# tum-vision/dvo_slam

Measured on AMD Instinct MI355X. Metric: frame-pair alignments/s (640x480, 4-level pyramid) + finest-level HBM GB/s vs roofline, higher is better.
Workload: dtype f32 (Gram operands exact f16 hi + lo pairs on every level, f32 accumulate); 1 GPU; 1024 pairs (BASELINE config 4): independent 640x480 RGB-D frame pairs, seeds 0..1023, pair i on rank i mod 1, 4-level pyramid, FirstLevel=3, LastLevel=0, MaxIterationsPerLevel=100, Precision=5e-7, Mu=0; step = every rank re-ingests the raw planes of its shard from HBM (pyramids, sampling planes, point selection) and aligns it as one batch; the build of step k+1 (build stream) overlaps the match of; pairs=1024, pairs_per_gpu=1024, width=640, height=480, lanes=1 lane

## Files before the change

dvo_slam_amd/csrc/align_coarse.hip:

```cpp
#include "fast_sweep.h"
#include "mfma_sweep.h"
#include "solver_logic.h"

namespace dvo_hip {

namespace {

__device__ __forceinline__ int coarse_uniform(int v) { return __builtin_amdgcn_readfirstlane(v); }
__device__ __forceinline__ float coarse_uniform(float v) { return __builtin_bit_cast(float, __builtin_amdgcn_readfirstlane(__builtin_bit_cast(int, v))); }

template <typename T>
__device__ __forceinline__ void coarse_copy(T* dst, const T* src) {
  static_assert(sizeof(T) % 4 == 0, "POD must be a multiple of 4 bytes");
  const unsigned* s = reinterpret_cast<const unsigned*>(src);
  unsigned* d = reinterpret_cast<unsigned*>(dst);
  for (int i = threadIdx.x; i < int(sizeof(T) / 4); i += kBlock) d[i] = s[i];
}

constexpr int kCoarseReduceInFlight = 8;
constexpr int kCoarseLlSlots = 4, kCoarseLlLoads = 4;

}

template <int WG_PER_CU>
// ... 37 lines not shown
    const int tiles = g.tiles_x * g.tiles_y;
    const bool window_level = !g.linear && g.compact;
    float* my_partials = a.partials + size_t(pair) * a.max_tiles * kAccStride;
    float2* my_residuals = a.scratch + size_t(pair) * a.max_entries;
    int* my_flag = a.f16_range_flag ? a.f16_range_flag + pair : nullptr;

    for (;;) {
      float KT[12], Pp[4];
#pragma unroll
      for (int i = 0; i < 12; ++i) KT[i] = coarse_uniform(st.KT[i]);
#pragma unroll
      for (int i = 0; i < 4; ++i) Pp[i] = coarse_uniform(st.P_prev[i]);
      const bool first = coarse_uniform(st.first) != 0;
      if (window_level) {
        const FastWeights wt(Pp, first);
        if (g.w % kTileW != 0) {
#pragma unroll 1
          for (int tile = 0; tile < tiles; ++tile)
            fast_sweep_tile<2, true, true, 0, false>(g, KT, wt, pp, 0, tile, my_partials, my_residuals, lds, no_table, a.fallback_count, my_flag);
        } else {
#pragma unroll 1
          for (int tile = 0; tile < tiles; ++tile)
            fast_sweep_tile<2, false, true, 0, false>(g, KT, wt, pp, 0, tile, my_partials, my_residuals, lds, no_table, a.fallback_count, my_flag);
        }
      } else if (g.linear) {
#pragma unroll 1
        for (int tile = 0; tile < tiles; ++tile) {
          mfma_sweep_tile<kCoarseRowsPerWave, true, 2>(g, KT, Pp, first, pp, 0, tile, my_partials, my_residuals, &slab[0][0], counts, my_flag);
          __syncthreads();
        }
      } else {
#pragma unroll 1
        for (int tile = 0; tile < tiles; ++tile) {
          mfma_sweep_tile<kCoarseRowsPerWave, false, 2>(g, KT, Pp, first, pp, 0, tile, my_partials, my_residuals, &slab[0][0], counts, my_flag);
          __syncthreads();
        }
      }
      __syncthreads();
// ... 78 lines not shown
```

dvo_slam_amd/csrc/align_fast.hip:

```cpp
#include "fast_sweep.h"
#include "solver_step.h"

namespace dvo_hip {

template <int STORE, bool PARTIAL, bool COMPACT, int COMPAT, bool HI_J, int TAIL>
__global__ __launch_bounds__(256, COMPAT == 2 ? 4 : 5) void k_sweep_fast(
    const LevelGeom g, const PairPtrs* __restrict__ pairs, const PairState* __restrict__ states, int n_pairs,
    float* __restrict__ partials, float2* __restrict__ scratch, int blocks_per_xcd, unsigned long long* __restrict__ fallback_count, int* __restrict__ f16_range_flag,
    const SolverStepArgs tail) {
  const int tiles = g.tiles_x * g.tiles_y;
  const int total = tiles * n_pairs;
  const int xcd = blockIdx.x & 7, slot = blockIdx.x >> 3;
  const int item = xcd * blocks_per_xcd + slot;
  if (item >= total) return;
  const int entry = item / tiles, tile = item - entry * tiles;
  const int pair = pair_of_launch_index(g, entry);
  if (pair < 0) return;
  const PairState& st = states[pair];
  __shared__ __attribute__((aligned(16))) float slab[4][kSlabFloatsF16];
  __shared__ __attribute__((aligned(16))) float2 win[kFastCells];
  __shared__ __attribute__((aligned(16))) int bbox[4][2];
  __shared__ int counts[4];
  static_assert(TAIL == 0 || sizeof(SweepTailLds) + 16 <= sizeof(win), "the step's LDS lies over the window");
  if (!st.active || st.level != g.level) {
// ... 5 lines not shown
  const FastRcpSource rcp_table = {__builtin_amdgcn_make_buffer_rsrc(const_cast<float*>(COMPAT ? g.rcp_table : nullptr), 0, COMPAT ? (4 << (23 - g.rcp_shift)) : 0, 0x00020000),
                                   rcp_lds, g.rcp_shift};
  if constexpr (COMPAT == 2) {
    const int entries = 1 << (23 - g.rcp_shift);
    const __amdgpu_buffer_rsrc_t packed = __builtin_amdgcn_make_buffer_rsrc(const_cast<float*>(g.rcp_table) + entries, 0, entries * 2, 0x00020000);
    f32x4 chunk[2];
#pragma unroll
    for (int j = 0; j < 2; ++j) chunk[j] = __builtin_bit_cast(f32x4, __builtin_amdgcn_raw_buffer_load_b128(packed, (int(threadIdx.x) + j * 256) * 16, 0, 0));
#pragma unroll
    for (int j = 0; j < 2; ++j)
      if ((int(threadIdx.x) + j * 256) * 8 < entries) reinterpret_cast<f32x4*>(rcp_lds)[threadIdx.x + j * 256] = chunk[j];
    __syncthreads();
  }
  const FastLds lds = {slab, win, bbox, counts};
  const FastWeights wt(st);
  fast_sweep_tile<STORE, PARTIAL, COMPACT, COMPAT, HI_J, TAIL != 0>(g, st.KT, wt, pp, pair, tile, partials, scratch, lds, rcp_table, fallback_count, f16_range_flag);
  if constexpr (TAIL == 1) sweep_tail(g, tail, pair, reinterpret_cast<char*>(win));
  if constexpr (TAIL == 2) sweep_tail_wide(g, tail, pair, reinterpret_cast<char*>(win));
}

bool sweep_fast_has_tail(int variant, const LevelGeom& g) { return variant == 8 && !g.rcp_table && !g.gram_hi_j && fast_sweep_supports(g); }

bool fast_sweep_takes_width(int w) { return w >= kFastCols && w % 2 == 0; }

bool fast_sweep_supports(const LevelGeom& g) {
  const long long plane_bytes = 8ll * g.w * g.h, packed_bytes = 8ll * kCompactTileEntries * g.tiles_x * g.tiles_y;
  return !g.linear && fast_sweep_takes_width(g.w) && g.w < 32768 && g.h < 32768 && plane_bytes < (1ll << 31) && packed_bytes < (1ll << 31);
}

void launch_sweep_fast(hipStream_t s, int variant, const LevelGeom& g, const PairPtrs* pairs, const PairState* states, int n_pairs,
                       float* partials, float2* scratch, unsigned long long* fallback_count, int* f16_range_flag, const SolverStepArgs* tail) {
  const int total = g.tiles_x * g.tiles_y * n_pairs;
  const int per_xcd = (total + 7) / 8;
  const dim3 grid(per_xcd * 8), block(256);
  const bool partial = g.w % kTileW != 0, compact = g.compact != 0;
  const SolverStepArgs no_tail = {};
  if (tail) {
    auto with = [&](auto partial_tag, auto compact_tag) {
      constexpr bool kP = decltype(partial_tag)::value, kC = decltype(compact_tag)::value;
      if (tail->pair_sums) k_sweep_fast<2, kP, kC, 0, false, 2><<<grid, block, 0, s>>>(g, pairs, states, n_pairs, partials, scratch, per_xcd, fallback_count, f16_range_flag, *tail);
      else k_sweep_fast<2, kP, kC, 0, false, 1><<<grid, block, 0, s>>>(g, pairs, states, n_pairs, partials, scratch, per_xcd, fallback_count, f16_range_flag, *tail);
    };
    if (compact) { if (partial) with(std::true_type{}, std::true_type{}); else with(std::false_type{}, std::true_type{}); }
    else { if (partial) with(std::true_type{}, std::false_type{}); else with(std::false_type{}, std::false_type{}); }
    return;
  }
  auto go = [&](auto store_tag, auto partial_tag, auto compact_tag, auto compat_tag) {
    constexpr int kStore = decltype(store_tag)::value;
    if (g.gram_hi_j && kStore == 2)
      k_sweep_fast<2, decltype(partial_tag)::value, decltype(compact_tag)::value, decltype(compat_tag)::value, true, 0>
          <<<grid, block, 0, s>>>(g, pairs, states, n_pairs, partials, scratch, per_xcd, fallback_count, f16_range_flag, no_tail);
    else
      k_sweep_fast<kStore, decltype(partial_tag)::value, decltype(compact_tag)::value, decltype(compat_tag)::value, false, 0>
          <<<grid, block, 0, s>>>(g, pairs, states, n_pairs, partials, scratch, per_xcd, fallback_count, f16_range_flag, no_tail);
  };
  using S1 = std::integral_constant<int, 1>;
  using S2 = std::integral_constant<int, 2>;
  using T = std::true_type;
  using F = std::false_type;
  using C0 = std::integral_constant<int, 0>;
  using C1 = std::integral_constant<int, 1>;
  using C2 = std::integral_constant<int, 2>;
  if (g.rcp_table && g.rcp_packed) {
    if (compact) { if (partial) go(S2{}, T{}, T{}, C2{}); else go(S2{}, F{}, T{}, C2{}); }
    else { if (partial) go(S2{}, T{}, F{}, C2{}); else go(S2{}, F{}, F{}, C2{}); }
  } else if (g.rcp_table) {
    if (compact) { if (partial) go(S2{}, T{}, T{}, C1{}); else go(S2{}, F{}, T{}, C1{}); }
    else { if (partial) go(S2{}, T{}, F{}, C1{}); else go(S2{}, F{}, F{}, C1{}); }
  } else if (variant == 8) {
    if (compact) { if (partial) go(S2{}, T{}, T{}, C0{}); else go(S2{}, F{}, T{}, C0{}); }
    else { if (partial) go(S2{}, T{}, F{}, C0{}); else go(S2{}, F{}, F{}, C0{}); }
  } else {
    if (compact) { if (partial) go(S1{}, T{}, T{}, C0{}); else go(S1{}, F{}, T{}, C0{}); }
    else { if (partial) go(S1{}, T{}, F{}, C0{}); else go(S1{}, F{}, F{}, C0{}); }
  }
}

}
```

dvo_slam_amd/csrc/capi_frames.inc:

```
int stamp_build(dvo_hip_context* ctx, int n, dvo_hip_frame* const* frames) {
  const unsigned long long seq = ++ctx->build_seq;
  DVO_HIP_TRY(ctx, hipEventRecord(ctx->build_events[seq % dvo_hip_context::kBuildRing], ctx->build_stream));
  for (int i = 0; i < n; ++i) frames[i]->built_seq = seq;
  return DVO_HIP_OK;
}

int wait_for_ticket(dvo_hip_context* ctx, unsigned long long need, bool upload) {
  unsigned long long& waited = upload ? ctx->upload_waited_seq : ctx->main_waited_seq;
  hipStream_t stream = upload ? ctx->upload_stream : ctx->stream;
  if (need <= waited) return DVO_HIP_OK;
  const unsigned long long oldest_live = ctx->build_seq >= dvo_hip_context::kBuildRing ? ctx->build_seq - dvo_hip_context::kBuildRing + 1 : 1;
  const unsigned long long use = need < oldest_live ? oldest_live : need;
  DVO_HIP_TRY(ctx, hipStreamWaitEvent(stream, ctx->build_events[use % dvo_hip_context::kBuildRing], 0));
  waited = use;
  return DVO_HIP_OK;
}

int wait_for_build(dvo_hip_context* ctx, int n, dvo_hip_frame* const* frames) {
  unsigned long long need = 0;
  for (int i = 0; i < n; ++i)
    if (frames[i] && frames[i]->built_seq > need) need = frames[i]->built_seq;
  return wait_for_ticket(ctx, need, false);
}

// ... 95 lines not shown
    off += align_up(size_t(c->h[l]) * 4, 256);
    e = hipMemcpy(c->tx[l], host.data(), size_t(c->w[l]) * 4, hipMemcpyHostToDevice);
    if (e == hipSuccess) e = hipMemcpy(c->ty[l], host.data() + c->w[l], size_t(c->h[l]) * 4, hipMemcpyHostToDevice);
    if (e != hipSuccess) {
      c->tables.release();
      delete c;
      ctx->err = std::string("hipMemcpy(camera tables): ") + hipGetErrorString(e);
      return DVO_HIP_ERR_HIP;
    }
  }
  ctx->cameras.push_back(c);
  *out = c;
  return DVO_HIP_OK;
}

void level_tiles(int w, int h, int rows_per_wave, bool linear, int* tiles_x, int* tiles_y) {
  const int th = kWavesPerBlock * rows_per_wave;
  if (linear) {
    const int segments = (w * h + kTileW - 1) / kTileW;
    *tiles_x = 1;
    *tiles_y = (segments + th - 1) / th;
  } else {
    *tiles_x = (w + kTileW - 1) / kTileW;
    *tiles_y = (h + th - 1) / th;
  }
}

bool level_uses_fast_window(const dvo_hip_context* ctx, int w, int h) {
  return ctx->opt_variant >= 8 && fast_sweep_takes_width(w) && w < 32768 && h < 32768;
}

bool level_uses_small(const dvo_hip_context* ctx, int w, int h);

bool level_is_linear(const dvo_hip_context* ctx, int w) { return ctx->opt_variant >= 5 && w % kTileW != 0 && !level_uses_fast_window(ctx, w, 4); }

bool level_uses_window(const dvo_hip_context* ctx, int w, int h) {
  return (ctx->opt_variant >= 6 && w % kTileW == 0 && w < 32768 && h < 32768) || level_uses_fast_window(ctx, w, h);
}
// ... 1 lines not shown
bool level_uses_small(const dvo_hip_context* ctx, int w, int h) {
  return ctx->opt_small_sweep && ctx->opt_variant >= 8 && !ctx->opt_ref_compat && !ctx->opt_ref_order && !level_uses_window(ctx, w, h) && level_is_linear(ctx, w) && small_sweep_takes(w, h);
}

LevelGeom make_geom(const dvo_hip_context* ctx, const CameraGeom* cam, int level, int rows_per_wave) {
  LevelGeom g;
  g.w = cam->w[level]; g.h = cam->h[level];
  g.fx = cam->K[level][0]; g.fy = cam->K[level][1]; g.ox = cam->K[level][2]; g.oy = cam->K[level][3];
  g.wi_x = 0.5f * g.fx / 255.0f; g.wi_y = 0.5f * g.fy / 255.0f;
  g.half_wi_x = 0.5f * g.wi_x; g.half_wi_y = 0.5f * g.wi_y; g.half_fx = 0.5f * g.fx; g.half_fy = 0.5f * g.fy;
  g.tx = cam->tx[level]; g.ty = cam->ty[level];
  g.level = level;
  g.pair_list = nullptr;
  g.skip_flags = nullptr;
  g.linear = level_is_linear(ctx, g.w) ? 1 : 0;
  level_tiles(g.w, g.h, rows_per_wave, g.linear != 0, &g.tiles_x, &g.tiles_y);
  g.rcp_table = ctx->opt_ref_compat ? ctx->rcp_table.as<float>() : nullptr;
  g.rcp_shift = ctx->rcp_shift;
  g.rcp_packed = ctx->opt_ref_compat == 1 ? ctx->rcp_packed : 0;
  g.gram_hi_j = !ctx->opt_gram_lo_parts && !ctx->opt_deterministic && !ctx->opt_ref_compat && ctx->opt_variant == 8 && size_t(g.w) * g.h >= 150000 ? 1 : 0;
  g.small = level_uses_small(ctx, g.w, g.h) ? 1 : 0;
  g.compact = ctx->opt_compact_residuals && !ctx->opt_ref_order && ctx->opt_variant >= 8 && rows_per_wave == 4 && fast_sweep_supports(g) ? 1 : 0;
  return g;
}

int pick_rows_per_wave(const dvo_hip_context* ctx, const CameraGeom* cam, int level, int n_pairs) {
  if (level_uses_window(ctx, cam->w[level], cam->h[level])) return 4;
  if (level_uses_small(ctx, cam->w[level], cam->h[level]) && ctx->opt_rows_per_wave == 0) {
    const int tiles = ctx->opt_small_tiles > 0 ? ctx->opt_small_tiles : BatchPolicy(ctx->compute_units).small_level_tiles(n_pairs);
    const int segments = (cam->w[level] * cam->h[level] + kTileW - 1) / kTileW;
    const int rows = (segments + kWavesPerBlock * tiles - 1) / (kWavesPerBlock * tiles);
// ... 448 lines not shown
```

dvo_slam_amd/csrc/device_types.h:

```cpp
#pragma once

#include <stdint.h>

#include "hd_compat.h"
#include "lens.h"
#include "depth_rig.h"
#include "cloud_map.h"
#include "cloud_colour.h"
#include "map_render.h"

#include "../../include/dvo_hip.h"

namespace dvo_hip {

constexpr int kMaxLevels = DVO_HIP_MAX_LEVELS;
constexpr int kBlock = 256;
constexpr int kWavesPerBlock = 4;
constexpr int kTileW = 64;

constexpr int kAccN = 0, kAccS = 1, kAccJ00 = 4, kAccJ11 = 25, kAccJ01 = 46, kAccB00 = 67, kAccB01 = 73, kAccB11 = 79;
constexpr int kNumAcc = 85;
constexpr int kAccStride = 88;

struct LevelGeom {
  int w, h;
  float fx, fy, ox, oy;
  float wi_x, wi_y;
  float half_wi_x, half_wi_y, half_fx, half_fy;
  const float* tx;
  const float* ty;
  int tiles_x, tiles_y;
  int linear;
  const float* rcp_table;
  int rcp_shift;
  int rcp_packed;
  int compact;
  int small;
  int gram_hi_j;
  int level;
  const int* pair_list;
  const unsigned char* skip_flags;
};

DVO_HD int pair_of_launch_index(const LevelGeom& g, int k) {
  const int pair = g.pair_list ? g.pair_list[k] : k;
  return pair >= 0 && g.skip_flags && g.skip_flags[pair] ? -1 : pair;
}

struct PairPtrs;
struct NextLevel {
  int valid;
  int level;
  float fx, fy, ox, oy;
  const PairPtrs* pairs;
// ... 255 lines not shown
```

dvo_slam_amd/csrc/fast_sweep.h:

```cpp
#pragma once
#include <type_traits>

#include "gram_f16.h"


namespace dvo_hip {

constexpr int kFastTileRows = 16;
constexpr int kFastPitch = 96;
constexpr int kFastCols = 84;
constexpr int kFastPairs = kFastCols / 2;
constexpr int kFastRows = 28;
constexpr int kFastRowGroups = 6;
constexpr int kFastLoads = (kFastRows + kFastRowGroups - 1) / kFastRowGroups;
constexpr int kFastCells = kFastPitch * kFastRows;

typedef short __attribute__((ext_vector_type(2))) fast_i16x2;
typedef unsigned __attribute__((ext_vector_type(2))) fast_u32x2;
typedef unsigned __attribute__((__vector_size__(2 * sizeof(unsigned)))) fast_u32v2;
typedef const volatile __attribute__((address_space(3))) f32x2* FastLdsCellPtr;

__device__ __forceinline__ void fast_wave_min2max2_lane63(int& a, int& b, int& c, int& d) {
#define DVO_STAGE(ctrl)                                                                                            \
  asm volatile("s_nop 1\n\t"                                                                                       \
               "v_min_i32_dpp %0, %0, %0 " ctrl "\n\t"                                                              \
               "v_min_i32_dpp %1, %1, %1 " ctrl "\n\t"                                                              \
               "v_max_i32_dpp %2, %2, %2 " ctrl "\n\t"                                                              \
               "v_max_i32_dpp %3, %3, %3 " ctrl                                                                     \
               : "+v"(a), "+v"(b), "+v"(c), "+v"(d));
  DVO_STAGE("row_shr:1 row_mask:0xf bank_mask:0xf")
// ... 45 lines not shown
    }
    r = fast_rcp_host<COMPAT>(table, qz);
  } else {
    qz = fmaf(z, fmaf(KT[9], ty, c2), KT[11]);
    r = __builtin_amdgcn_rcpf(qz);
  }
  u = qx * r;
  v = qy * r;
}

struct FastWindow {
  int x0, y0, ww, wh;
  bool all_in;
};

__device__ __forceinline__ FastWindow fast_window_of(const int (*bbox)[2]) {
  fast_i16x2 lo = __builtin_bit_cast(fast_i16x2, bbox[0][0]), hi = __builtin_bit_cast(fast_i16x2, bbox[0][1]);
#pragma unroll
  for (int w4 = 1; w4 < 4; ++w4) {
    lo = __builtin_elementwise_min(lo, __builtin_bit_cast(fast_i16x2, bbox[w4][0]));
    hi = __builtin_elementwise_max(hi, __builtin_bit_cast(fast_i16x2, bbox[w4][1]));
  }
  const int lo_s = __builtin_amdgcn_readfirstlane(__builtin_bit_cast(int, lo)), hi_s = __builtin_amdgcn_readfirstlane(__builtin_bit_cast(int, hi));
  const int bu0 = lo_s & 0xffff, bv0 = (lo_s >> 16) & 0xffff, bu1 = hi_s & 0xffff, bv1 = (hi_s >> 16) & 0xffff;
  FastWindow wnd;
  wnd.x0 = (bu0 - 1) & ~1; wnd.y0 = bv0 - 1;
  const bool any = bu0 != 0x7fff;
  wnd.ww = any ? min(bu1 + 3 - wnd.x0, kFastCols) : 0;
  wnd.wh = any ? min(bv1 + 3 - wnd.y0, kFastRows) : 0;
  wnd.all_in = !any || (bu1 + 3 - wnd.x0 <= kFastCols && bv1 + 3 - wnd.y0 <= kFastRows);
  return wnd;
}

__device__ __forceinline__ void fast_fill_window(const LevelGeom& g, __amdgpu_buffer_rsrc_t curC, float2* win, const FastWindow& wnd, int row_bytes) {
  const int t = threadIdx.x;
  const int rg = t / kFastPairs, cxp = t - rg * kFastPairs;
  f32x4* dst = reinterpret_cast<f32x4*>(win) + rg * (kFastPitch / 2) + cxp;
  const int x0 = wnd.x0, y0 = wnd.y0, wh = wnd.wh;
  const bool interior = x0 >= 0 && x0 + kFastCols <= g.w && y0 >= 0 && y0 + kFastRows <= g.h;
  if (rg < kFastRowGroups && 2 * cxp < wnd.ww) {
    if (interior) {
      const int voff = (y0 + rg) * row_bytes + (x0 + 2 * cxp) * 8;
      const int voff_last = rg + (kFastLoads - 1) * kFastRowGroups < kFastRows ? voff : 0x7ffffff0;
      f32x4 cell[kFastLoads];
#pragma unroll
      for (int j = 0; j < kFastLoads; ++j)
        if (j * kFastRowGroups < wh)
          cell[j] = __builtin_bit_cast(f32x4, __builtin_amdgcn_raw_buffer_load_b128(curC, j == kFastLoads - 1 ? voff_last : voff, j * kFastRowGroups * row_bytes, 0));
#pragma unroll
// ... 12 lines not shown
      if (x < 0) {
#pragma unroll
        for (int j = 0; j < kFastLoads; ++j) { cell[j].z = cell[j].x; cell[j].w = cell[j].y; }
      }
      if (x >= g.w) {
#pragma unroll
        for (int j = 0; j < kFastLoads; ++j) { cell[j].x = cell[j].z; cell[j].y = cell[j].w; }
      }
#pragma unroll
      for (int j = 0; j < kFastLoads; ++j)
        if (rg + j * kFastRowGroups < kFastRows) dst[j * kFastRowGroups * (kFastPitch / 2)] = cell[j];
    }
  }
}

template <bool CHECKED, int COMPAT>
__device__ __forceinline__ void fast_fetch_cells(const LevelGeom& g, const FastRcpSource& table, const float* KT, __amdgpu_buffer_rsrc_t curC, const float2* win,
                                                 const FastWindow& wnd, int neg_base, const FastRow& r, bool ok, float tx, float ty, f32x2 (&P)[4][4],
                                                 unsigned& n_fallback) {
  if constexpr (!CHECKED) {
    const int addr = (r.idx << 3) + neg_base;
    FastLdsCellPtr q = (FastLdsCellPtr)(reinterpret_cast<const char*>(win) + (ok ? addr : 0));
#pragma unroll
    for (int rr = 0; rr < 4; ++rr)
#pragma unroll
      for (int cc = 0; cc < 4; ++cc)
        if ((rr == 1 || rr == 2) || (cc == 1 || cc == 2)) P[rr][cc] = q[rr * kFastPitch + cc];
  } else {
    float pu, pv, pqz;
    fast_project<COMPAT>(g, table, KT, fmaf(KT[0], tx, KT[2]), fmaf(KT[4], tx, KT[6]), fmaf(KT[8], tx, KT[10]), r.z, tx, ty, pu, pv, pqz);
    const int u0 = int(pu), v0 = int(pv);
    const int cx = u0 - wnd.x0 - 1, cy = v0 - wnd.y0 - 1;
    const bool in_win = ok && unsigned(cx) <= unsigned(kFastCols - 4) && unsigned(cy) <= unsigned(kFastRows - 4);
    FastLdsCellPtr q = (FastLdsCellPtr)(win + (in_win ? cy * kFastPitch + cx : 0));
// ... 215 lines not shown
  const unsigned long long lanes = __ballot(n_fallback != 0);
  if (lanes) {
    unsigned t = n_fallback;
    for (int off = 32; off > 0; off >>= 1) t += __shfl_down(t, off, 64);
    if (lane == 0) atomicAdd(fallback_count, (unsigned long long)t);
  }
}

struct FastLds {
  float (*slab)[kSlabFloatsF16];
  float2* win;
  int (*bbox)[2];
  int* counts;
};

template <int STORE, bool PARTIAL, bool COMPACT, int COMPAT, bool HI_J, bool WT = false>
__device__ __forceinline__ void fast_sweep_tile(const LevelGeom& g, const float* KT, const FastWeights& wt, const PairPtrs& pp, int pair, int tile,
                                                float* __restrict__ partials, float2* __restrict__ scratch, const FastLds& lds,
                                                const FastRcpSource& rcp_table, unsigned long long* __restrict__ fallback_count,
                                                int* __restrict__ f16_range_flag) {
  constexpr int RPW = kFastTileRows / 4;
  const int tiles = g.tiles_x * g.tiles_y;
  const int tile_x = tile % g.tiles_x, tile_y = tile / g.tiles_x;
  const int plane_bytes = g.w * g.h * 8;
  const __amdgpu_buffer_rsrc_t refR = __builtin_amdgcn_make_buffer_rsrc(const_cast<float2*>(pp.refR), 0, plane_bytes, 0x00020000);
  const __amdgpu_buffer_rsrc_t curC = __builtin_amdgcn_make_buffer_rsrc(const_cast<float2*>(pp.curC), 0, plane_bytes, 0x00020000);
  const __amdgpu_buffer_rsrc_t resid = COMPACT ? __builtin_amdgcn_make_buffer_rsrc(scratch + size_t(pair) * tiles * kCompactTileEntries, 0, tiles * kCompactTileEntries * 8, 0x00020000)
                                               : __builtin_amdgcn_make_buffer_rsrc(scratch + size_t(pair) * size_t(g.w) * g.h, 0, plane_bytes, 0x00020000);
  const __amdgpu_buffer_rsrc_t resid_none = __builtin_amdgcn_make_buffer_rsrc(scratch, 0, 0, 0x00020000);
  const int lane = threadIdx.x & 63, wave = __builtin_amdgcn_readfirstlane(threadIdx.x >> 6);
  const unsigned gram_entries = kGramEntryTable.e[min(int(threadIdx.x), kNumAcc - 1)];
  const int u_r = PARTIAL ? min(tile_x * kTileW + lane, g.w - 1) : tile_x * kTileW + lane;
  const unsigned long long col_mask = PARTIAL ? __builtin_amdgcn_ballot_w64(tile_x * kTileW + lane < g.w) : ~0ull;
  const int row_bytes = g.w * 8;
  const float tx_u = g.tx[u_r];
  const float cx_u = fmaf(tx_u, tx_u, 1.0f);

  float (*slab)[kSlabFloatsF16] = lds.slab;
  float2* win = lds.win;
  int (*bbox)[2] = lds.bbox;
  int* counts = lds.counts;
  float* my = slab[wave];
  const int off_px = u_r * 8;
  const int off_store = !PARTIAL || tile_x * kTileW + lane < g.w ? off_px : plane_bytes;
  const int off_edge = (lane == 0 ? max(u_r - 1, 0) : lane == 63 ? min(u_r + 1, g.w - 1) : u_r) * 8 + 4;

  const int row0 = tile_y * kFastTileRows + wave;
  float ty_rows[RPW];
#pragma unroll
  for (int k = 0; k < RPW; ++k) ty_rows[k] = g.ty[min(row0 + k * 4, g.h - 1)];

  FastRow rs[RPW];
  unsigned long long ok_row[RPW];
  int umin = 0x7fff, vmin = 0x7fff, umax = 0, vmax = 0;
  {
    const float c0 = fmaf(KT[0], tx_u, KT[2]), c1 = fmaf(KT[4], tx_u, KT[6]), c2 = fmaf(KT[8], tx_u, KT[10]);
    const unsigned w2_bits = __builtin_bit_cast(unsigned, float(g.w - 2)), h2_bits = __builtin_bit_cast(unsigned, float(g.h - 2));
    float zv[RPW], iv[RPW], up[RPW], down[RPW], edge[RPW];
#pragma unroll
    for (int k = 0; k < RPW; ++k) {
      const int v = min(row0 + k * 4, g.h - 1);
      const int soff = v * row_bytes;
      const f32x2 zi = __builtin_bit_cast(f32x2, __builtin_amdgcn_raw_buffer_load_b64(refR, off_px, soff, 0));
      zv[k] = zi.x;
      iv[k] = zi.y;
      up[k] = __builtin_bit_cast(float, __builtin_amdgcn_raw_buffer_load_b32(refR, off_px + 4, soff - (v > 0 ? row_bytes : 0), 0));
      down[k] = __builtin_bit_cast(float, __builtin_amdgcn_raw_buffer_load_b32(refR, off_px + 4, soff + (v < g.h - 1 ? row_bytes : 0), 0));
      edge[k] = __builtin_bit_cast(float, __builtin_amdgcn_raw_buffer_load_b32(refR, off_edge, soff, 0));
    }
#pragma unroll
    for (int k = 0; k < RPW; ++k) {
      const int v_r = row0 + k * 4;
      const int ic = __builtin_bit_cast(int, iv[k]), ie = __builtin_bit_cast(int, edge[k]);
      const float right = __builtin_bit_cast(float, __builtin_amdgcn_update_dpp(ie, ic, 0x130, 0xf, 0xf, false));
      const float left = __builtin_bit_cast(float, __builtin_amdgcn_update_dpp(ie, ic, 0x138, 0xf, 0xf, false));
      const float z = zv[k];
      float u, v, qz;
      fast_project<COMPAT>(g, rcp_table, KT, c0, c1, c2, z, tx_u, ty_rows[k], u, v, qz);
      const unsigned long long ok_mask = v_r < g.h ? __builtin_amdgcn_ballot_w64(__builtin_bit_cast(unsigned, u) <= w2_bits) &
                                                         __builtin_amdgcn_ballot_w64(__builtin_bit_cast(unsigned, v) <= h2_bits) & col_mask : 0ull;
      const bool ok = __builtin_amdgcn_inverse_ballot_w64(ok_mask);
      const int u0 = int(u), v0 = int(v);
      rs[k].z = z;
      rs[k].i = iv[k];
      rs[k].gx = right - left;
      rs[k].gy = down[k] - up[k];
      rs[k].qz = qz;
      rs[k].a1 = __builtin_amdgcn_fractf(u);
      rs[k].b1 = __builtin_amdgcn_fractf(v);
      rs[k].idx = int(__umul24(v0, kFastPitch)) + u0;
      ok_row[k] = ok_mask;
      if (ok) {
        umin = min(umin, u0); umax = max(umax, u0);
        vmin = min(vmin, v0); vmax = max(vmax, v0);
      }
    }
  }
  fast_wave_min2max2_lane63(umin, vmin, umax, vmax);
  if (lane == 63) {
    bbox[wave][0] = umin | (vmin << 16); bbox[wave][1] = umax | (vmax << 16);
  }
  __syncthreads();
  const FastWindow wnd = fast_window_of(bbox);

  fast_fill_window(g, curC, win, wnd, row_bytes);
  __syncthreads();

  const int neg_base = -8 * ((wnd.x0 + 1) + kFastPitch * (wnd.y0 + 1));
  f32x4 acc0 = {0.0f, 0.0f, 0.0f, 0.0f}, acc1 = {0.0f, 0.0f, 0.0f, 0.0f};
  int n_valid = 0;
  unsigned n_fallback = 0;
  auto sweep_row = [&](int k, auto checked_tag) __attribute__((always_inline)) {
    constexpr bool CHECKED = decltype(checked_tag)::value;
    const int v_r = row0 + k * 4;
    f32x2 P[4][4];
    fast_fetch_cells<CHECKED, COMPAT>(g, rcp_table, KT, curC, win, wnd, neg_base, rs[k], __builtin_amdgcn_inverse_ballot_w64(ok_row[k]), tx_u, ty_rows[k], P, n_fallback);
    if constexpr (COMPACT)
      fast_row_tail<STORE, true, COMPAT, HI_J, WT ? 16 : 0>(g, rcp_table, P, rs[k], ok_row[k], tx_u, ty_rows[k], cx_u, wt, resid, 0, (tile * kCompactTileEntries + wave * kCompactWaveEntries) * 8, my, lane, acc0, acc1, n_valid);
    else
      fast_row_tail<STORE, false, COMPAT, HI_J, WT ? 16 : 0>(g, rcp_table, P, rs[k], ok_row[k], tx_u, ty_rows[k], cx_u, wt, v_r < g.h ? resid : resid_none, off_store, v_r * row_bytes, my, lane, acc0, acc1, n_valid);
  };
  if (wnd.all_in) {
#pragma unroll
    for (int k = 0; k < RPW; ++k) sweep_row(k, std::false_type{});
  } else {
#pragma unroll
    for (int k = 0; k < RPW; ++k) sweep_row(k, std::true_type{});
  }

#pragma unroll
  for (int i = 0; i < 4; ++i) {
    my[((lane >> 4) * 4 + i) * 16 + (lane & 15)] = acc0[i];
    my[256 + ((lane >> 4) * 4 + i) * 16 + (lane & 15)] = acc1[i];
  }
  if (lane == 0) counts[wave] = n_valid;
// ... 7 lines not shown
```

dvo_slam_amd/csrc/launch.h:

```cpp
#pragma once

#include <hip/hip_runtime.h>

#include "device_types.h"

namespace dvo_hip {

struct RefOrderSeg;
struct RefOrderPair;
struct RefOrderPlane;

void launch_pyr_down(hipStream_t s, const FrameBuildPtrs* tbl, int n_frames, int level, int w, int h);
void launch_build_from_raw(hipStream_t s, const FrameBuildPtrs* tbl, int n_frames, float scale, int w0, int h0, int levels, int role, bool strips,
                           float ithr, float dthr, int max_workgroups, int cur_flavor = kCurAB, int c_levels = 0, int colour_channels = 0,
                           bool stream_nt = false, bool depth_f32 = false);
bool derive_strips_supports(int w);
void launch_derive_strips(hipStream_t s, const FrameBuildPtrs* tbl, int n_frames, int level, int w, int h, int role, float ithr, float dthr,
                          int max_workgroups, int cur_flavor, bool stream_nt = false);
bool ingest_strips_supports(int w0, bool wide, bool f32_image = false);
bool f32_strips_aligned(const void* plane, size_t pitch);
bool colour_strips_aligned(const void* colour, size_t pitch, int channels);
void launch_ingest_strips(hipStream_t s, const FrameBuildPtrs* tbl, int n_frames, float scale, int w0, int h0, int levels, int role,
                          float ithr, float dthr, int max_workgroups, int cur_flavor, int c_levels, int colour_channels = 0, bool stream_nt = false,
                          bool depth_f32 = false);
// ... 60 lines not shown
                        size_t stage_bytes);

void launch_residual_reduce(hipStream_t s, int variant, int rows_per_wave, bool finest_level, const LevelGeom& g, const PairPtrs* pairs,
                            const PairState* states, int n_pairs, float* partials, float2* scratch, unsigned long long* window_fallbacks = nullptr,
                            int* f16_range_flag = nullptr, const SolverStepArgs* tail = nullptr);
bool sweep_has_tail(int variant, int rows_per_wave, const LevelGeom& g);
bool sweep_fast_has_tail(int variant, const LevelGeom& g);
bool mfma_sweep_has_tail(int variant, int rows_per_wave, const LevelGeom& g);
void launch_residual_reduce_mfma(hipStream_t s, int rows_per_wave, bool finest_level, const LevelGeom& g, const PairPtrs* pairs,
                                 const PairState* states, int n_pairs, float* partials, float2* scratch, int mode = 0,
                                 int* f16_range_flag = nullptr, const SolverStepArgs* tail = nullptr);
bool window_sweep_supports(const LevelGeom& g);
void launch_sweep_window(hipStream_t s, bool f16, const LevelGeom& g, const PairPtrs* pairs, const PairState* states, int n_pairs,
                         float* partials, float2* scratch, unsigned long long* fallback_count, int* f16_range_flag = nullptr);
bool fast_sweep_takes_width(int w);
bool fast_sweep_supports(const LevelGeom& g);
void launch_sweep_fast(hipStream_t s, int variant, const LevelGeom& g, const PairPtrs* pairs, const PairState* states, int n_pairs,
                       float* partials, float2* scratch, unsigned long long* fallback_count, int* f16_range_flag = nullptr,
                       const SolverStepArgs* tail = nullptr);
bool small_sweep_takes(int w, int h);
void launch_sweep_small(hipStream_t s, int rows_per_wave, const LevelGeom& g, const PairPtrs* pairs, const PairState* states, int n_pairs,
                        float* partials, float2* scratch, int* f16_range_flag = nullptr);
void launch_stream_mix(hipStream_t s, const PairPtrs* pairs, int n_pairs, int n_px, float2* scratch, float* sink, bool window_planes = false);
void launch_loglik(hipStream_t s, const LevelGeom& g, const PairState* states, int n_pairs, const float* partials,
                   const float2* scratch, double* ll_partials, int blocks_per_pair, bool one_schedule = false, const RefOrderPair* ref_order = nullptr);

void launch_ref_order(hipStream_t s, const LevelGeom& g, const PairState* states, int n_pairs, const float2* scratch, RefOrderSeg* rows, RefOrderPair* out);
void launch_ref_order_drop_last(hipStream_t s, const RefOrderPlane* planes, int n_planes);
void launch_ref_order_restore(hipStream_t s, const RefOrderPlane* planes, int n_planes);

// ... 28 lines not shown
```

Before: 92820 alignments/s.

## Add 32-column tile shape to fast window sweep for narrow levels

Introduces a FastShape template so the contracted window sweep can use 32-column tiles, with two sub-rows per wave, on levels whose width is a multiple of 32 but not 64. Tile geometry, window size, fill layout and neighbour handling at the sub-row edges are parameterised, and the launch and coarse kernels dispatch on g.tile_cols. The aim is to avoid partial 64-wide tiles and wasted lanes on widths like 160 or 80 in the 640x480 pyramid. The cost is more template instantiations, extra edge selects and per-lane row addressing in the narrow shape.

```diff
diff --git a/dvo_slam_amd/csrc/align_coarse.hip b/dvo_slam_amd/csrc/align_coarse.hip
--- a/dvo_slam_amd/csrc/align_coarse.hip
+++ b/dvo_slam_amd/csrc/align_coarse.hip
@@ -75,14 +75,18 @@
       const bool first = coarse_uniform(st.first) != 0;
       if (window_level) {
         const FastWeights wt(Pp, first);
-        if (g.w % kTileW != 0) {
+        if (g.tile_cols == 32) {
 #pragma unroll 1
           for (int tile = 0; tile < tiles; ++tile)
-            fast_sweep_tile<2, true, true, 0, false>(g, KT, wt, pp, 0, tile, my_partials, my_residuals, lds, no_table, a.fallback_count, my_flag);
+            fast_sweep_tile<32, 2, false, true, 0, false>(g, KT, wt, pp, 0, tile, my_partials, my_residuals, lds, no_table, a.fallback_count, my_flag);
+        } else if (g.w % kTileW != 0) {
+#pragma unroll 1
+          for (int tile = 0; tile < tiles; ++tile)
+            fast_sweep_tile<64, 2, true, true, 0, false>(g, KT, wt, pp, 0, tile, my_partials, my_residuals, lds, no_table, a.fallback_count, my_flag);
         } else {
 #pragma unroll 1
           for (int tile = 0; tile < tiles; ++tile)
-            fast_sweep_tile<2, false, true, 0, false>(g, KT, wt, pp, 0, tile, my_partials, my_residuals, lds, no_table, a.fallback_count, my_flag);
+            fast_sweep_tile<64, 2, false, true, 0, false>(g, KT, wt, pp, 0, tile, my_partials, my_residuals, lds, no_table, a.fallback_count, my_flag);
         }
       } else if (g.linear) {
 #pragma unroll 1
diff --git a/dvo_slam_amd/csrc/align_fast.hip b/dvo_slam_amd/csrc/align_fast.hip
--- a/dvo_slam_amd/csrc/align_fast.hip
+++ b/dvo_slam_amd/csrc/align_fast.hip
@@ -3,7 +3,7 @@
 
 namespace dvo_hip {
 
-template <int STORE, bool PARTIAL, bool COMPACT, int COMPAT, bool HI_J, int TAIL>
+template <int COLS, int STORE, bool PARTIAL, bool COMPACT, int COMPAT, bool HI_J, int TAIL>
 __global__ __launch_bounds__(256, COMPAT == 2 ? 4 : 5) void k_sweep_fast(
     const LevelGeom g, const PairPtrs* __restrict__ pairs, const PairState* __restrict__ states, int n_pairs,
     float* __restrict__ partials, float2* __restrict__ scratch, int blocks_per_xcd, unsigned long long* __restrict__ fallback_count, int* __restrict__ f16_range_flag,
@@ -43,18 +43,37 @@
   }
   const FastLds lds = {slab, win, bbox, counts};
   const FastWeights wt(st);
-  fast_sweep_tile<STORE, PARTIAL, COMPACT, COMPAT, HI_J, TAIL != 0>(g, st.KT, wt, pp, pair, tile, partials, scratch, lds, rcp_table, fallback_count, f16_range_flag);
+  fast_sweep_tile<COLS, STORE, PARTIAL, COMPACT, COMPAT, HI_J, TAIL != 0>(g, st.KT, wt, pp, pair, tile, partials, scratch, lds, rcp_table, fallback_count, f16_range_flag);
   if constexpr (TAIL == 1) sweep_tail(g, tail, pair, reinterpret_cast<char*>(win));
   if constexpr (TAIL == 2) sweep_tail_wide(g, tail, pair, reinterpret_cast<char*>(win));
 }
 
 bool sweep_fast_has_tail(int variant, const LevelGeom& g) { return variant == 8 && !g.rcp_table && !g.gram_hi_j && fast_sweep_supports(g); }
 
-bool fast_sweep_takes_width(int w) { return w >= kFastCols && w % 2 == 0; }
+bool fast_sweep_takes_width(int w) { return fast_shape_takes_width(w); }
+
+int fast_sweep_level_cols(int w, int h) { return 8ll * w * h < (1ll << 30) ? fast_sweep_cols(w) : kTileW; }
 
 bool fast_sweep_supports(const LevelGeom& g) {
   const long long plane_bytes = 8ll * g.w * g.h, packed_bytes = 8ll * kCompactTileEntries * g.tiles_x * g.tiles_y;
   return !g.linear && fast_sweep_takes_width(g.w) && g.w < 32768 && g.h < 32768 && plane_bytes < (1ll << 31) && packed_bytes < (1ll << 31);
+}
+
+namespace {
+
+template <int COLS, bool PARTIAL>
+struct FastShapeTag {
+  static constexpr int cols = COLS;
+  static constexpr bool partial = PARTIAL;
+};
+
+template <class F>
+void with_shape(const LevelGeom& g, F&& f) {
+  if (g.tile_cols == 32) f(FastShapeTag<32, false>{});
+  else if (g.w % kTileW != 0) f(FastShapeTag<64, true>{});
+  else f(FastShapeTag<64, false>{});
+}
+
 }
 
 void launch_sweep_fast(hipStream_t s, int variant, const LevelGeom& g, const PairPtrs* pairs, const PairState* states, int n_pairs,
@@ -62,47 +81,49 @@
   const int total = g.tiles_x * g.tiles_y * n_pairs;
   const int per_xcd = (total + 7) / 8;
   const dim3 grid(per_xcd * 8), block(256);
-  const bool partial = g.w % kTileW != 0, compact = g.compact != 0;
+  const bool compact = g.compact != 0;
   const SolverStepArgs no_tail = {};
+  auto launch = [&](auto shape, auto store_tag, auto compact_tag, auto compat_tag, auto hi_j_tag, auto tail_tag, const SolverStepArgs& step) {
+    constexpr int kCols = decltype(shape)::cols, kStore = decltype(store_tag)::value, kCompat = decltype(compat_tag)::value, kTail = decltype(tail_tag)::value;
+    constexpr bool kC = decltype(compact_tag)::value, kHiJ = decltype(hi_j_tag)::value;
+    k_sweep_fast<kCols, kStore, decltype(shape)::partial, kC, kCompat, kHiJ, kTail><<<grid, block, 0, s>>>(g, pairs, states, n_pairs, partials, scratch, per_xcd, fallback_count, f16_range_flag, step);
+  };
+  using I0 = std::integral_constant<int, 0>;
+  using I1 = std::integral_constant<int, 1>;
+  using I2 = std::integral_constant<int, 2>;
   if (tail) {
-    auto with = [&](auto partial_tag, auto compact_tag) {
-      constexpr bool kP = decltype(partial_tag)::value, kC = decltype(compact_tag)::value;
-      if (tail->pair_sums) k_sweep_fast<2, kP, kC, 0, false, 2><<<grid, block, 0, s>>>(g, pairs, states, n_pairs, partials, scratch, per_xcd, fallback_count, f16_range_flag, *tail);
-      else k_sweep_fast<2, kP, kC, 0, false, 1><<<grid, block, 0, s>>>(g, pairs, states, n_pairs, partials, scratch, per_xcd, fallback_count, f16_range_flag, *tail);
+    auto with = [&](auto shape, auto compact_tag) {
+      if (tail->pair_sums) launch(shape, I2{}, compact_tag, I0{}, std::false_type{}, I2{}, *tail);
+      else launch(shape, I2{}, compact_tag, I0{}, std::false_type{}, I1{}, *tail);
     };
-    if (compact) { if (partial) with(std::true_type{}, std::true_type{}); else with(std::false_type{}, std::true_type{}); }
-    else { if (partial) with(std::true_type{}, std::false_type{}); else with(std::false_type{}, std::false_type{}); }
+    with_shape(g, [&](auto shape) {
+      if (compact) with(shape, std::true_type{});
+      else with(shape, std::false_type{});
+    });
     return;
   }
-  auto go = [&](auto store_tag, auto partial_tag, auto compact_tag, auto compat_tag) {
-    constexpr int kStore = decltype(store_tag)::value;
-    if (g.gram_hi_j && kStore == 2)
-      k_sweep_fast<2, decltype(partial_tag)::value, decltype(compact_tag)::value, decltype(compat_tag)::value, true, 0>
-          <<<grid, block, 0, s>>>(g, pairs, states, n_pairs, partials, scratch, per_xcd, fallback_count, f16_range_flag, no_tail);
-    else
-      k_sweep_fast<kStore, decltype(partial_tag)::value, decltype(compact_tag)::value, decltype(compat_tag)::value, false, 0>
-          <<<grid, block, 0, s>>>(g, pairs, states, n_pairs, partials, scratch, per_xcd, fallback_count, f16_range_flag, no_tail);
+  auto go = [&](auto store_tag, auto shape, auto compact_tag, auto compat_tag) {
+    if (g.gram_hi_j && decltype(store_tag)::value == 2) launch(shape, I2{}, compact_tag, compat_tag, std::true_type{}, I0{}, no_tail);
+    else launch(shape, store_tag, compact_tag, compat_tag, std::false_type{}, I0{}, no_tail);
   };
-  using S1 = std::integral_constant<int, 1>;
-  using S2 = std::integral_constant<int, 2>;
+  using S1 = I1;
+  using S2 = I2;
   using T = std::true_type;
   using F = std::false_type;
-  using C0 = std::integral_constant<int, 0>;
-  using C1 = std::integral_constant<int, 1>;
-  using C2 = std::integral_constant<int, 2>;
-  if (g.rcp_table && g.rcp_packed) {
-    if (compact) { if (partial) go(S2{}, T{}, T{}, C2{}); else go(S2{}, F{}, T{}, C2{}); }
-    else { if (partial) go(S2{}, T{}, F{}, C2{}); else go(S2{}, F{}, F{}, C2{}); }
-  } else if (g.rcp_table) {
-    if (compact) { if (partial) go(S2{}, T{}, T{}, C1{}); else go(S2{}, F{}, T{}, C1{}); }
-    else { if (partial) go(S2{}, T{}, F{}, C1{}); else go(S2{}, F{}, F{}, C1{}); }
-  } else if (variant == 8) {
-    if (compact) { if (partial) go(S2{}, T{}, T{}, C0{}); else go(S2{}, F{}, T{}, C0{}); }
-    else { if (partial) go(S2{}, T{}, F{}, C0{}); else go(S2{}, F{}, F{}, C0{}); }
-  } else {
-    if (compact) { if (partial) go(S1{}, T{}, T{}, C0{}); else go(S1{}, F{}, T{}, C0{}); }
-    else { if (partial) go(S1{}, T{}, F{}, C0{}); else go(S1{}, F{}, F{}, C0{}); }
-  }
+  using C0 = I0;
+  using C1 = I1;
+  using C2 = I2;
+  with_shape(g, [&](auto shape) {
+    if (g.rcp_table && g.rcp_packed) {
+      if (compact) go(S2{}, shape, T{}, C2{}); else go(S2{}, shape, F{}, C2{});
+    } else if (g.rcp_table) {
+      if (compact) go(S2{}, shape, T{}, C1{}); else go(S2{}, shape, F{}, C1{});
+    } else if (variant == 8) {
+      if (compact) go(S2{}, shape, T{}, C0{}); else go(S2{}, shape, F{}, C0{});
+    } else {
+      if (compact) go(S1{}, shape, T{}, C0{}); else go(S1{}, shape, F{}, C0{});
+    }
+  });
 }
 
 }
diff --git a/dvo_slam_amd/csrc/capi_frames.inc b/dvo_slam_amd/csrc/capi_frames.inc
--- a/dvo_slam_amd/csrc/capi_frames.inc
+++ b/dvo_slam_amd/csrc/capi_frames.inc
@@ -133,14 +133,14 @@
   return DVO_HIP_OK;
 }
 
-void level_tiles(int w, int h, int rows_per_wave, bool linear, int* tiles_x, int* tiles_y) {
-  const int th = kWavesPerBlock * rows_per_wave;
+void level_tiles(int w, int h, int rows_per_wave, bool linear, int* tiles_x, int* tiles_y, int tile_cols = kTileW) {
+  const int th = kWavesPerBlock * rows_per_wave * (kTileW / tile_cols);
   if (linear) {
     const int segments = (w * h + kTileW - 1) / kTileW;
     *tiles_x = 1;
     *tiles_y = (segments + th - 1) / th;
   } else {
-    *tiles_x = (w + kTileW - 1) / kTileW;
+    *tiles_x = (w + tile_cols - 1) / tile_cols;
     *tiles_y = (h + th - 1) / th;
   }
 }
@@ -172,7 +172,8 @@
   g.pair_list = nullptr;
   g.skip_flags = nullptr;
   g.linear = level_is_linear(ctx, g.w) ? 1 : 0;
-  level_tiles(g.w, g.h, rows_per_wave, g.linear != 0, &g.tiles_x, &g.tiles_y);
+  g.tile_cols = !g.linear && rows_per_wave == 4 && level_uses_fast_window(ctx, g.w, g.h) ? fast_sweep_level_cols(g.w, g.h) : kTileW;
+  level_tiles(g.w, g.h, rows_per_wave, g.linear != 0, &g.tiles_x, &g.tiles_y, g.tile_cols);
   g.rcp_table = ctx->opt_ref_compat ? ctx->rcp_table.as<float>() : nullptr;
   g.rcp_shift = ctx->rcp_shift;
   g.rcp_packed = ctx->opt_ref_compat == 1 ? ctx->rcp_packed : 0;
diff --git a/dvo_slam_amd/csrc/device_types.h b/dvo_slam_amd/csrc/device_types.h
--- a/dvo_slam_amd/csrc/device_types.h
+++ b/dvo_slam_amd/csrc/device_types.h
@@ -38,6 +38,7 @@
   int small;
   int gram_hi_j;
   int level;
+  int tile_cols;
   const int* pair_list;
   const unsigned char* skip_flags;
 };
diff --git a/dvo_slam_amd/csrc/fast_shape.h b/dvo_slam_amd/csrc/fast_shape.h
--- /dev/null
+++ b/dvo_slam_amd/csrc/fast_shape.h
@@ -0,0 +1,45 @@
+#pragma once
+
+#include "hd_compat.h"
+
+namespace dvo_hip {
+
+constexpr int kFastLanes = 64;
+constexpr int kFastWaves = 4, kFastWaveRows = 4;
+
+template <int COLS>
+struct FastShape {
+  static_assert(COLS == 64 || COLS == 32, "tile widths of the contracted window sweep");
+  static constexpr int cols = COLS;
+  static constexpr int sub = kFastLanes / COLS;
+  static constexpr int tile_rows = kFastWaves * kFastWaveRows * sub;
+  static constexpr int win_cols = COLS + 20, win_rows = tile_rows + 12;
+  static constexpr int pitch = COLS == 64 ? 96 : 60;
+  static constexpr int pairs = win_cols / 2;
+  static constexpr int row_groups = 256 / pairs;
+  static constexpr int loads = (win_rows + row_groups - 1) / row_groups;
+  static constexpr int cells = pitch * win_rows;
+  static_assert(pitch % 2 == 0 && win_cols % 2 == 0 && pitch >= win_cols, "a 16-byte store holds two cells");
+};
+
+constexpr int kFastCells = FastShape<64>::cells;
+static_assert(FastShape<64>::cells == 2688 && FastShape<32>::cells == 2640, "the window's cells, shape by shape");
+static_assert(FastShape<32>::cells <= kFastCells, "every shape's window fits the one array");
+static_assert(FastShape<64>::loads * FastShape<64>::row_groups >= FastShape<64>::win_rows && FastShape<32>::loads * FastShape<32>::row_groups >= FastShape<32>::win_rows, "the fill covers the window");
+
+DVO_HD int fast_sweep_cols(int w) { return w % 64 == 0 ? 64 : w % 32 == 0 && w >= 32 + 20 ? 32 : 64; }
+DVO_HD int fast_sweep_tile_rows(int cols) { return kFastWaves * kFastWaveRows * (kFastLanes / cols); }
+DVO_HD bool fast_shape_takes_width(int w) { return w % 2 == 0 && w >= fast_sweep_cols(w) + 20; }
+DVO_HD int fast_sweep_tiles_x(int w) { const int c = fast_sweep_cols(w); return (w + c - 1) / c; }
+DVO_HD int fast_sweep_tiles_y(int w, int h) { const int r = fast_sweep_tile_rows(fast_sweep_cols(w)); return (h + r - 1) / r; }
+
+template <int COLS>
+DVO_HD int fast_lane_col(int lane) { return lane % COLS; }
+template <int COLS>
+DVO_HD int fast_lane_x(int tile_x, int lane) { return tile_x * COLS + fast_lane_col<COLS>(lane); }
+template <int COLS>
+DVO_HD int fast_lane_y(int tile_y, int wave, int k, int lane) {
+  return tile_y * FastShape<COLS>::tile_rows + (k * kFastWaves + wave) * FastShape<COLS>::sub + lane / COLS;
+}
+
+}
diff --git a/dvo_slam_amd/csrc/fast_sweep.h b/dvo_slam_amd/csrc/fast_sweep.h
--- a/dvo_slam_amd/csrc/fast_sweep.h
+++ b/dvo_slam_amd/csrc/fast_sweep.h
@@ -1,19 +1,11 @@
 #pragma once
 #include <type_traits>
 
+#include "fast_shape.h"
 #include "gram_f16.h"
 
 
 namespace dvo_hip {
-
-constexpr int kFastTileRows = 16;
-constexpr int kFastPitch = 96;
-constexpr int kFastCols = 84;
-constexpr int kFastPairs = kFastCols / 2;
-constexpr int kFastRows = 28;
-constexpr int kFastRowGroups = 6;
-constexpr int kFastLoads = (kFastRows + kFastRowGroups - 1) / kFastRowGroups;
-constexpr int kFastCells = kFastPitch * kFastRows;
 
 typedef short __attribute__((ext_vector_type(2))) fast_i16x2;
 typedef unsigned __attribute__((ext_vector_type(2))) fast_u32x2;
@@ -89,6 +81,7 @@
   bool all_in;
 };
 
+template <class S>
 __device__ __forceinline__ FastWindow fast_window_of(const int (*bbox)[2]) {
   fast_i16x2 lo = __builtin_bit_cast(fast_i16x2, bbox[0][0]), hi = __builtin_bit_cast(fast_i16x2, bbox[0][1]);
 #pragma unroll
@@ -101,13 +94,15 @@
   FastWindow wnd;
   wnd.x0 = (bu0 - 1) & ~1; wnd.y0 = bv0 - 1;
   const bool any = bu0 != 0x7fff;
-  wnd.ww = any ? min(bu1 + 3 - wnd.x0, kFastCols) : 0;
-  wnd.wh = any ? min(bv1 + 3 - wnd.y0, kFastRows) : 0;
-  wnd.all_in = !any || (bu1 + 3 - wnd.x0 <= kFastCols && bv1 + 3 - wnd.y0 <= kFastRows);
+  wnd.ww = any ? min(bu1 + 3 - wnd.x0, S::win_cols) : 0;
+  wnd.wh = any ? min(bv1 + 3 - wnd.y0, S::win_rows) : 0;
+  wnd.all_in = !any || (bu1 + 3 - wnd.x0 <= S::win_cols && bv1 + 3 - wnd.y0 <= S::win_rows);
   return wnd;
 }
 
+template <class S>
 __device__ __forceinline__ void fast_fill_window(const LevelGeom& g, __amdgpu_buffer_rsrc_t curC, float2* win, const FastWindow& wnd, int row_bytes) {
+  constexpr int kFastPairs = S::pairs, kFastPitch = S::pitch, kFastCols = S::win_cols, kFastRows = S::win_rows, kFastRowGroups = S::row_groups, kFastLoads = S::loads;
   const int t = threadIdx.x;
   const int rg = t / kFastPairs, cxp = t - rg * kFastPairs;
   f32x4* dst = reinterpret_cast<f32x4*>(win) + rg * (kFastPitch / 2) + cxp;
@@ -150,10 +145,11 @@
   }
 }
 
-template <bool CHECKED, int COMPAT>
+template <class S, bool CHECKED, int COMPAT>
 __device__ __forceinline__ void fast_fetch_cells(const LevelGeom& g, const FastRcpSource& table, const float* KT, __amdgpu_buffer_rsrc_t curC, const float2* win,
                                                  const FastWindow& wnd, int neg_base, const FastRow& r, bool ok, float tx, float ty, f32x2 (&P)[4][4],
                                                  unsigned& n_fallback) {
+  constexpr int kFastPitch = S::pitch, kFastCols = S::win_cols, kFastRows = S::win_rows;
   if constexpr (!CHECKED) {
     const int addr = (r.idx << 3) + neg_base;
     FastLdsCellPtr q = (FastLdsCellPtr)(reinterpret_cast<const char*>(win) + (ok ? addr : 0));
@@ -399,12 +395,14 @@
   int* counts;
 };
 
-template <int STORE, bool PARTIAL, bool COMPACT, int COMPAT, bool HI_J, bool WT = false>
+template <int COLS, int STORE, bool PARTIAL, bool COMPACT, int COMPAT, bool HI_J, bool WT = false>
 __device__ __forceinline__ void fast_sweep_tile(const LevelGeom& g, const float* KT, const FastWeights& wt, const PairPtrs& pp, int pair, int tile,
                                                 float* __restrict__ partials, float2* __restrict__ scratch, const FastLds& lds,
                                                 const FastRcpSource& rcp_table, unsigned long long* __restrict__ fallback_count,
                                                 int* __restrict__ f16_range_flag) {
-  constexpr int RPW = kFastTileRows / 4;
+  using S = FastShape<COLS>;
+  constexpr int RPW = kFastWaveRows, SUB = S::sub;
+  static_assert(!PARTIAL || COLS == 64, "a narrow tile is only chosen where it divides the width");
   const int tiles = g.tiles_x * g.tiles_y;
   const int tile_x = tile % g.tiles_x, tile_y = tile / g.tiles_x;
   const int plane_bytes = g.w * g.h * 8;
@@ -415,8 +413,9 @@
   const __amdgpu_buffer_rsrc_t resid_none = __builtin_amdgcn_make_buffer_rsrc(scratch, 0, 0, 0x00020000);
   const int lane = threadIdx.x & 63, wave = __builtin_amdgcn_readfirstlane(threadIdx.x >> 6);
   const unsigned gram_entries = kGramEntryTable.e[min(int(threadIdx.x), kNumAcc - 1)];
-  const int u_r = PARTIAL ? min(tile_x * kTileW + lane, g.w - 1) : tile_x * kTileW + lane;
-  const unsigned long long col_mask = PARTIAL ? __builtin_amdgcn_ballot_w64(tile_x * kTileW + lane < g.w) : ~0ull;
+  const int col = fast_lane_col<COLS>(lane), u_lane = fast_lane_x<COLS>(tile_x, lane);
+  const int u_r = PARTIAL ? min(u_lane, g.w - 1) : u_lane;
+  const unsigned long long col_mask = PARTIAL ? __builtin_amdgcn_ballot_w64(u_lane < g.w) : ~0ull;
   const int row_bytes = g.w * 8;
   const float tx_u = g.tx[u_r];
   const float cx_u = fmaf(tx_u, tx_u, 1.0f);
@@ -427,13 +426,13 @@
   int* counts = lds.counts;
   float* my = slab[wave];
   const int off_px = u_r * 8;
-  const int off_store = !PARTIAL || tile_x * kTileW + lane < g.w ? off_px : plane_bytes;
-  const int off_edge = (lane == 0 ? max(u_r - 1, 0) : lane == 63 ? min(u_r + 1, g.w - 1) : u_r) * 8 + 4;
-
-  const int row0 = tile_y * kFastTileRows + wave;
+  const int off_store = !PARTIAL || u_lane < g.w ? off_px : plane_bytes;
+  const int off_edge = (col == 0 ? max(u_r - 1, 0) : col == COLS - 1 ? min(u_r + 1, g.w - 1) : u_r) * 8 + 4;
+
+  auto row_of = [&](int k) { return fast_lane_y<COLS>(tile_y, wave, k, lane); };
   float ty_rows[RPW];
 #pragma unroll
-  for (int k = 0; k < RPW; ++k) ty_rows[k] = g.ty[min(row0 + k * 4, g.h - 1)];
+  for (int k = 0; k < RPW; ++k) ty_rows[k] = g.ty[min(row_of(k), g.h - 1)];
 
   FastRow rs[RPW];
   unsigned long long ok_row[RPW];
@@ -444,26 +443,43 @@
     float zv[RPW], iv[RPW], up[RPW], down[RPW], edge[RPW];
 #pragma unroll
     for (int k = 0; k < RPW; ++k) {
-      const int v = min(row0 + k * 4, g.h - 1);
+      const int v = min(row_of(k), g.h - 1);
       const int soff = v * row_bytes;
-      const f32x2 zi = __builtin_bit_cast(f32x2, __builtin_amdgcn_raw_buffer_load_b64(refR, off_px, soff, 0));
+      f32x2 zi;
+      if constexpr (SUB == 1) {
+        zi = __builtin_bit_cast(f32x2, __builtin_amdgcn_raw_buffer_load_b64(refR, off_px, soff, 0));
+        up[k] = __builtin_bit_cast(float, __builtin_amdgcn_raw_buffer_load_b32(refR, off_px + 4, soff - (v > 0 ? row_bytes : 0), 0));
+        down[k] = __builtin_bit_cast(float, __builtin_amdgcn_raw_buffer_load_b32(refR, off_px + 4, soff + (v < g.h - 1 ? row_bytes : 0), 0));
+        edge[k] = __builtin_bit_cast(float, __builtin_amdgcn_raw_buffer_load_b32(refR, off_edge, soff, 0));
+      } else {
+        zi = __builtin_bit_cast(f32x2, __builtin_amdgcn_raw_buffer_load_b64(refR, soff + off_px, 0, 0));
+        up[k] = __builtin_bit_cast(float, __builtin_amdgcn_raw_buffer_load_b32(refR, soff + off_px + 4 - (v > 0 ? row_bytes : 0), 0, 0));
+        down[k] = __builtin_bit_cast(float, __builtin_amdgcn_raw_buffer_load_b32(refR, soff + off_px + 4 + (v < g.h - 1 ? row_bytes : 0), 0, 0));
+        edge[k] = __builtin_bit_cast(float, __builtin_amdgcn_raw_buffer_load_b32(refR, soff + off_edge, 0, 0));
+      }
       zv[k] = zi.x;
       iv[k] = zi.y;
-      up[k] = __builtin_bit_cast(float, __builtin_amdgcn_raw_buffer_load_b32(refR, off_px + 4, soff - (v > 0 ? row_bytes : 0), 0));
-      down[k] = __builtin_bit_cast(float, __builtin_amdgcn_raw_buffer_load_b32(refR, off_px + 4, soff + (v < g.h - 1 ? row_bytes : 0), 0));
-      edge[k] = __builtin_bit_cast(float, __builtin_amdgcn_raw_buffer_load_b32(refR, off_edge, soff, 0));
     }
 #pragma unroll
     for (int k = 0; k < RPW; ++k) {
-      const int v_r = row0 + k * 4;
+      const int v_r = row_of(k);
       const int ic = __builtin_bit_cast(int, iv[k]), ie = __builtin_bit_cast(int, edge[k]);
-      const float right = __builtin_bit_cast(float, __builtin_amdgcn_update_dpp(ie, ic, 0x130, 0xf, 0xf, false));
-      const float left = __builtin_bit_cast(float, __builtin_amdgcn_update_dpp(ie, ic, 0x138, 0xf, 0xf, false));
+      float right = __builtin_bit_cast(float, __builtin_amdgcn_update_dpp(ie, ic, 0x130, 0xf, 0xf, false));
+      float left = __builtin_bit_cast(float, __builtin_amdgcn_update_dpp(ie, ic, 0x138, 0xf, 0xf, false));
+      if constexpr (SUB > 1) {
+        right = col == COLS - 1 ? edge[k] : right;
+        left = col == 0 ? edge[k] : left;
+      }
       const float z = zv[k];
       float u, v, qz;
       fast_project<COMPAT>(g, rcp_table, KT, c0, c1, c2, z, tx_u, ty_rows[k], u, v, qz);
-      const unsigned long long ok_mask = v_r < g.h ? __builtin_amdgcn_ballot_w64(__builtin_bit_cast(unsigned, u) <= w2_bits) &
-                                                         __builtin_amdgcn_ballot_w64(__builtin_bit_cast(unsigned, v) <= h2_bits) & col_mask : 0ull;
+      unsigned long long ok_mask;
+      if constexpr (SUB == 1)
+        ok_mask = v_r < g.h ? __builtin_amdgcn_ballot_w64(__builtin_bit_cast(unsigned, u) <= w2_bits) &
+                                  __builtin_amdgcn_ballot_w64(__builtin_bit_cast(unsigned, v) <= h2_bits) & col_mask : 0ull;
+      else
+        ok_mask = __builtin_amdgcn_ballot_w64(__builtin_bit_cast(unsigned, u) <= w2_bits) & __builtin_amdgcn_ballot_w64(__builtin_bit_cast(unsigned, v) <= h2_bits) &
+                  __builtin_amdgcn_ballot_w64(v_r < g.h);
       const bool ok = __builtin_amdgcn_inverse_ballot_w64(ok_mask);
       const int u0 = int(u), v0 = int(v);
       rs[k].z = z;
@@ -473,7 +489,7 @@
       rs[k].qz = qz;
       rs[k].a1 = __builtin_amdgcn_fractf(u);
       rs[k].b1 = __builtin_amdgcn_fractf(v);
-      rs[k].idx = int(__umul24(v0, kFastPitch)) + u0;
+      rs[k].idx = int(__umul24(v0, S::pitch)) + u0;
       ok_row[k] = ok_mask;
       if (ok) {
         umin = min(umin, u0); umax = max(umax, u0);
@@ -486,24 +502,26 @@
     bbox[wave][0] = umin | (vmin << 16); bbox[wave][1] = umax | (vmax << 16);
   }
   __syncthreads();
-  const FastWindow wnd = fast_window_of(bbox);
-
-  fast_fill_window(g, curC, win, wnd, row_bytes);
+  const FastWindow wnd = fast_window_of<S>(bbox);
+
+  fast_fill_window<S>(g, curC, win, wnd, row_bytes);
   __syncthreads();
 
-  const int neg_base = -8 * ((wnd.x0 + 1) + kFastPitch * (wnd.y0 + 1));
+  const int neg_base = -8 * ((wnd.x0 + 1) + S::pitch * (wnd.y0 + 1));
   f32x4 acc0 = {0.0f, 0.0f, 0.0f, 0.0f}, acc1 = {0.0f, 0.0f, 0.0f, 0.0f};
   int n_valid = 0;
   unsigned n_fallback = 0;
   auto sweep_row = [&](int k, auto checked_tag) __attribute__((always_inline)) {
     constexpr bool CHECKED = decltype(checked_tag)::value;
-    const int v_r = row0 + k * 4;
+    const int v_r = row_of(k);
     f32x2 P[4][4];
-    fast_fetch_cells<CHECKED, COMPAT>(g, rcp_table, KT, curC, win, wnd, neg_base, rs[k], __builtin_amdgcn_inverse_ballot_w64(ok_row[k]), tx_u, ty_rows[k], P, n_fallback);
+    fast_fetch_cells<S, CHECKED, COMPAT>(g, rcp_table, KT, curC, win, wnd, neg_base, rs[k], __builtin_amdgcn_inverse_ballot_w64(ok_row[k]), tx_u, ty_rows[k], P, n_fallback);
     if constexpr (COMPACT)
       fast_row_tail<STORE, true, COMPAT, HI_J, WT ? 16 : 0>(g, rcp_table, P, rs[k], ok_row[k], tx_u, ty_rows[k], cx_u, wt, resid, 0, (tile * kCompactTileEntries + wave * kCompactWaveEntries) * 8, my, lane, acc0, acc1, n_valid);
+    else if constexpr (SUB == 1)
+      fast_row_tail<STORE, false, COMPAT, HI_J, WT ? 16 : 0>(g, rcp_table, P, rs[k], ok_row[k], tx_u, ty_rows[k], cx_u, wt, v_r < g.h ? resid : resid_none, off_store, v_r * row_bytes, my, lane, acc0, acc1, n_valid);
     else
-      fast_row_tail<STORE, false, COMPAT, HI_J, WT ? 16 : 0>(g, rcp_table, P, rs[k], ok_row[k], tx_u, ty_rows[k], cx_u, wt, v_r < g.h ? resid : resid_none, off_store, v_r * row_bytes, my, lane, acc0, acc1, n_valid);
+      fast_row_tail<STORE, false, COMPAT, HI_J, WT ? 16 : 0>(g, rcp_table, P, rs[k], ok_row[k], tx_u, ty_rows[k], cx_u, wt, resid, v_r < g.h ? v_r * row_bytes + off_store : plane_bytes, 0, my, lane, acc0, acc1, n_valid);
   };
   if (wnd.all_in) {
 #pragma unroll
diff --git a/dvo_slam_amd/csrc/launch.h b/dvo_slam_amd/csrc/launch.h
--- a/dvo_slam_amd/csrc/launch.h
+++ b/dvo_slam_amd/csrc/launch.h
@@ -98,6 +98,7 @@
 void launch_sweep_window(hipStream_t s, bool f16, const LevelGeom& g, const PairPtrs* pairs, const PairState* states, int n_pairs,
                          float* partials, float2* scratch, unsigned long long* fallback_count, int* f16_range_flag = nullptr);
 bool fast_sweep_takes_width(int w);
+int fast_sweep_level_cols(int w, int h);
 bool fast_sweep_supports(const LevelGeom& g);
 void launch_sweep_fast(hipStream_t s, int variant, const LevelGeom& g, const PairPtrs* pairs, const PairState* states, int n_pairs,
                        float* partials, float2* scratch, unsigned long long* fallback_count, int* f16_range_flag = nullptr,
```

Result: no change. 92210 alignments/s (median of 3 runs) (-0.7%).
